# lionl1106/Clip-Neural-image-conpression

Hardware: AMD Instinct MI355X
Metric: images/sec @256px 50-step DDIM, batch=8/GPU (higher is better)
Workload: dtype bf16; 1 GPU; 256px base=128 ch_mult=(1, 2, 2) 50-step DDIM (eta=0), batch=8/GPU, key-seeded synthetic weights (out.* x0.1), synthetic z / x_T; global_batch=8, parallelism=dp1 (independent batches, no collective in the loop), graph=hipGraph, one replay per step, steps_in_flight=1

## Files before the change

clip-neural-image-conpression_amd/csrc/ccn_api.hip:

```cpp
#include "../../include/ccn_hip.h"
#include "ccn_internal.h"

#include <algorithm>
#include <cmath>
#include <cstdio>
#include <cstdlib>
#include <cstring>
#include <functional>
#include <map>
#include <memory>
#include <string>
#include <vector>

using namespace ccn;

namespace {

thread_local std::string g_err;
int fail(int code, const std::string& msg) { g_err = msg; return code; }
#define HIPCHK(expr)                                                                                     \
    do {                                                                                                 \
        hipError_t e_ = (expr);                                                                          \
        if (e_ != hipSuccess)                                                                            \
            return fail(CCN_EHIP, std::string(#expr) + ": " + hipGetErrorString(e_));                    \
// ... 314 lines not shown
        std::vector<uint16_t> buf(n, 0);
        for (int t = 0; t < taps; ++t)
            for (int o = 0; o < cw.Cout; ++o)
                for (int i = 0; i < cw.Cin_pad; ++i) buf[((size_t)t * cw.Cout_pad + o) * cw.Cin_pad + i] = f2bf_host(at(t, o, i));
        return upload(h, buf.data(), n * 2, &cw.w);
    }
    std::vector<float> buf(n, 0.f);
    for (int t = 0; t < taps; ++t)
        for (int o = 0; o < cw.Cout; ++o)
            for (int i = 0; i < cw.Cin_pad; ++i) buf[((size_t)t * cw.Cout_pad + o) * cw.Cin_pad + i] = at(t, o, i);
    return upload(h, buf.data(), n * 4, &cw.w);
}

int pack_conv3(ccn_handle_s* h, ConvW& cw, const std::string& name)
{
    const float* w = h->host.at(name + ".weight").data();
    const int cke = conv_cin_chunk(h->cfg.dtype);
    cw.Cin_pad = (int)align_up(cw.Cin, cke);
    const int I = cw.Cin;
    int rc = pack_and_upload(h, cw, 9, [&](int t, int o, int i) { return i < I ? w[((size_t)o * I + i) * 9 + t] : 0.f; });
    if (rc) return rc;
    if (cw.kind == KIND_C3S2 && cw.BN == 128 && h->cfg.dtype == CCN_DTYPE_BF16) {
        const int nch = cw.Cin_pad / cke, n32 = cw.Cout_pad / 32, O = cw.Cout;
        std::vector<uint16_t> fr((size_t)nch * 5 * n32 * 2 * 4 * 64 * 8, 0);
        for (int o = 0; o < O; ++o)
            for (int i = 0; i < I; ++i)
                for (int ps = 0; ps < 10; ++ps) {
                    const int tp = prs2_tap(ps >> 1, ps & 1);
                    if (tp >= 0) fr[prs2_frag_index(ps >> 1, ps & 1, o, i, cw.Cout_pad)] = f2bf_host(w[((size_t)o * I + i) * 9 + tp]);
                }
        if ((rc = upload(h, fr.data(), fr.size() * 2, &cw.wfrag))) return rc;
    }
    if (cw.kind == KIND_C3S1 && cw.BN == 128 && h->cfg.dtype == CCN_DTYPE_BF16) {
        const int nch = cw.Cin_pad / cke, n32 = cw.Cout_pad / 32, O = cw.Cout;
        std::vector<uint16_t> fr((size_t)nch * n32 * 36 * 64 * 8, 0);
        for (int o = 0; o < O; ++o)
            for (int i = 0; i < I; ++i)
                for (int t = 0; t < 9; ++t) fr[pr3_frag_index(o, i, t, cw.Cout_pad)] = f2bf_host(w[((size_t)o * I + i) * 9 + t]);
        if ((rc = upload(h, fr.data(), fr.size() * 2, &cw.wfrag))) return rc;
    }
    return upload_f32(h, name + ".bias", &cw.bias);
}
int pack_convT(ccn_handle_s* h, ConvW& cw, const std::string& name)
{
    const float* w = h->host.at(name + ".weight").data();
    const int cke = conv_cin_chunk(h->cfg.dtype);
    cw.Cin_pad = (int)align_up(cw.Cin, cke);
    const int I = cw.Cin, O = cw.Cout;
    int rc = pack_and_upload(h, cw, 16, [&](int t, int o, int i) { return i < I ? w[((size_t)i * O + o) * 16 + t] : 0.f; });
    if (rc) return rc;
    if (cw.BN == 128 && h->cfg.dtype == CCN_DTYPE_BF16) {
        const int nch = cw.Cin_pad / cke, n32 = cw.Cout_pad / 32;
        std::vector<uint16_t> fr((size_t)4 * nch * n32 * 4 * 4 * 64 * 8, 0);
// ... 29 lines not shown
    }
    return upload_f32(h, name + ".bias", &cw.bias);
}

struct PlanBuilder {
    ccn_handle_s* h;
    Plan* plan;
    Bump bump;
    int B;
    int film_stride;
    PlanBuilder(ccn_handle_s* h_, Plan* p, void* ws, bool measure) : h(h_), plan(p), bump(ws, measure), B(p->B), film_stride(h_->F) {}

    TensorRef new_tensor(int C, int H, int W)
    {
        TensorRef t; t.C = C; t.H = H; t.W = W;
        t.p = bump.take((size_t)B * H * W * C * h->elem);
        return t;
    }
    float2* new_ab(int C) { return (float2*)bump.take((size_t)B * C * sizeof(float2)); }
    int groups_for(int C) const { return C < h->G ? C : h->G; }

    ConvRoute route(const ConvW& cw, int Hin, int Win, bool gn_ab, bool res, bool film) const
    {
        static const ConvPolicy policy{true, 128, false, !diag_env("CCN_NO_SPLITK"), diag_env("CCN_SPLITK_S1") != nullptr, true};
        return conv_route({h->cfg.dtype, cw.kind, false, cw.BN, cw.Cin, cw.Cin_pad, cw.Cout, cw.Cout_pad, B, Hin, Win, h->G, cw.wfrag != nullptr,
                           gn_ab, res, film}, policy);
    }

    void conv(const ConvW& cw, int family, const TensorRef& in, TensorRef& out, const float2* gn_ab, int film_off,
              const TensorRef* res, bool want_part, bool is_stem = false, bool is_head = false, const NormW* in_norm = nullptr)
    {
        const ConvRoute r = route(cw, in.H, in.W, gn_ab != nullptr, res != nullptr, film_off >= 0);
        const ConvGeom& g = r.g;
        std::shared_ptr<ConvArgs> ap(new ConvArgs());
        ConvArgs& a = *ap;
        r.fill(a);
        a.in = in.p; a.w = cw.w; a.wfrag = r.uses_frag() ? cw.wfrag : nullptr; a.bias = cw.bias; a.out = out.p;
        a.film = nullptr; a.res = res ? res->p : nullptr;
        static const bool no_instat = diag_env("CCN_NO_INSTAT") != nullptr;
        if (in_norm) {
            const int G_in = groups_for(cw.Cin), cpg_in = cw.Cin / G_in;
            if (r.gs_ok && !no_instat && in.C == cw.Cin && conv_in_kernel_stats(h->cfg.dtype, in.C, G_in, in.n_sp, in.bn)) {
                a.gs_part = in.part; a.gs_gamma = in_norm->gamma; a.gs_beta = in_norm->beta;
                a.gs_inv_count = 1.0 / ((double)cpg_in * in.H * in.W);
                a.gs_nsp = in.n_sp; a.gs_nnt = in.n_nt; a.gs_bn = in.bn; a.gs_cpg = cpg_in;
            } else gn_ab = gn(in, *in_norm);
        }
// ... 814 lines not shown
```

clip-neural-image-conpression_amd/csrc/ccn_conv_pr.hip:

```cpp
#include "ccn_device.h"
#include <cstdio>
#include <cstdlib>
#include <cstring>
#include <vector>
#include <algorithm>

namespace ccn {

namespace {

#define CCN_FDIV(x, m, d) ((m) ? (int)__umulhi((unsigned)(x), (m)) : (int)(x))

template <int TH_> struct PrLdsT {
    static constexpr int HROWS = TH_ + 2, HPITCH = 34;
    static constexpr int A_BYTES = HROWS * HPITCH * 128;
    static constexpr int SP = 272;
    static constexpr int STG_BYTES = TH_ * 32 * SP;
    static constexpr int CHS_BYTES = 4 * 128 * 2 * 4;
    static constexpr int TOTAL = 2 * A_BYTES + STG_BYTES + CHS_BYTES;
};
typedef PrLdsT<8> PrLds;
static_assert(PrLds::TOTAL <= 160 * 1024, "LDS budget");

}

template <int NTAPS, int D, int MODE, int TH = 8, int GS = 0, bool P4 = false>
__global__ __launch_bounds__(512) void conv_pr_kernel(const ConvArgs a, const int grid_tiles)
{
    static_assert(TH == 8 || (TH == 4 && NTAPS == 9), "4-row tiles: 3x3 stride-1 form only");
    static_assert(!P4 || (NTAPS == 4 && MODE != 2), "plane passes of 2x2 taps: the 4-tap consumers, no split-K");
    constexpr bool RES = MODE == 1;
    constexpr bool RR = MODE != 0;
    typedef __bf16 T;
    constexpr int MF = 4, NF = 2;
    constexpr int BN = 128;
    constexpr int HROWS = TH + 2;
    constexpr int OSC = (NTAPS == 4 && !P4) ? 2 : 1, NPARC = (NTAPS == 4 && !P4) ? 4 : 1;
    constexpr int EPC = 8, CKE = 64;
    constexpr int NSTEP = NTAPS * 4;
    constexpr bool S2 = NTAPS == 2;
    constexpr int NPASS = S2 ? 5 : (P4 ? 4 : 1);
    constexpr int IS = (S2 || P4) ? 2 : 1;
    static_assert(NSTEP % D == 0, "the register ring must wrap at the chunk boundary");
    using L = PrLdsT<TH>;
    constexpr int HPITCH = L::HPITCH;
    extern __shared__ __attribute__((aligned(16))) unsigned char smem[];
    unsigned char* const stg = smem + 2 * L::A_BYTES;

    const int tid = threadIdx.x, lane = tid & 63, wave = tid >> 6;
    const int r = lane & 31, h = lane >> 5;

    const int grid = (int)gridDim.x;
    const int vb = (grid & 7) == 0 ? ((int)blockIdx.x & 7) * (grid >> 3) + ((int)blockIdx.x >> 3) : (int)blockIdx.x;
    const int ntiles = grid_tiles;
    const int my_tiles = (ntiles - vb + grid - 1) / grid;
    auto vt = [&](int ti) __attribute__((always_inline)) { return vb + ti * grid; };
    const int ks = (MODE == 2 && a.ksplit == 2) ? 2 : 1;
    const unsigned xcc_id = MODE == 2 ? (unsigned)__builtin_amdgcn_s_getreg((3 << 11) | 20) : 0u;
    const int nck = a.nchunk / ks;
    const int ktotal = my_tiles * nck;
    auto vt_tile = [&](int v) __attribute__((always_inline)) { return ks == 2 ? (v >> 1) : v; };
    auto vt_kh = [&](int v) __attribute__((always_inline)) { return ks == 2 ? (v & 1) : 0; };

    const unsigned char* const inb = (const unsigned char*)a.in;
    constexpr bool gstat = GS == 1;
    static_assert(GS != 1 || (NTAPS == 9 && MODE != 2), "in-kernel statistics: 3x3 stride-1 layers without split-K");
// ... 282 lines not shown
            qn_bt[0] = *(const f32x4*)(a.gs_beta + q_cbs); qn_bt[1] = *(const f32x4*)(a.gs_beta + q_cbs + 4);
        } else gkn.load(a.gn_ab + (size_t)q_b * a.Cin + q_cbs, gn && q_cv);
    };
    auto coef_sel = [&]() __attribute__((always_inline)) {
        if (gstat) {
            const int src = CCN_FDIV(q_cbs, a.fd_gscpg, a.gs_cpg) * 8;
            qn_mean = __shfl(st_mean, src); qn_rstd = __shfl(st_rstd, src);
        }
    };
    auto prep = [&]() __attribute__((always_inline)) {
        const bool fresh = decode();
        coef_loads();
        if (fresh) { stats_issue(q_b); stats_reduce(); st_b = q_b; }
        coef_sel();
    };
    auto adopt = [&]() __attribute__((always_inline)) {
        if (gstat) gk.from_raw(qn_g, qn_bt, qn_mean, qn_rstd, gn && q_cv_i);
        else gk = gkn;
    };
    auto issue_loads = [&](int r0 = 0, int r1 = TH + 2, bool with_x = true) __attribute__((always_inline)) {
        const int b = __builtin_amdgcn_readfirstlane(q_b), iy0 = __builtin_amdgcn_readfirstlane(q_iy0), ix0 = __builtin_amdgcn_readfirstlane(q_ix0);
        const int cc = __builtin_amdgcn_readfirstlane(q_c / NPASS);
        const int pass = q_c - cc * NPASS;
        const int py = S2 ? (pass <= 2 ? 1 : 0) : (P4 ? (pass < 2 ? 1 : 0) : 0);
        const int px = S2 ? ((pass <= 1 || pass == 3) ? 1 : 0) : (P4 ? ((pass & 1) ? 0 : 1) : 0);
        const int cb = cc * CKE + ck * EPC;
        const bool cv = q_tv && cb < a.Cin;
        q_cv_i = cv;
        const unsigned img_bytes = (unsigned)(a.Hin * a.Win * a.Cin) * (unsigned)sizeof(T);
        const unsigned coff = (unsigned)(((q_tv && cc * CKE < a.Cin) ? cc : 0) * CKE) * (unsigned)sizeof(T);
        const auto srd = __builtin_amdgcn_make_buffer_rsrc((void*)(inb + (size_t)b * img_bytes + coff), 0, img_bytes - coff, 0x00020000);
        const int rs = IS * a.Win * a.Cin * (int)sizeof(T);
        const int ixr = IS * (ix0 + pcol) + px;
        colv = cv && ixr >= 0 && ixr < a.Win;
        const unsigned cmask = colv ? 0u : OOB;
        const int base = ((IS * iy0 + py) * a.Win + ixr) * a.Cin * (int)sizeof(T) + ck * 16;
        const int first = IS * iy0 + py;
        const int r_lo = first < 0 ? (-first + IS - 1) / IS : 0;
        int r_hi = (a.Hin - first + IS - 1) / IS; r_hi = r_hi > HROWS ? HROWS : (r_hi < 0 ? 0 : r_hi);
        rowm = q_tv ? (((1u << r_hi) - 1u) & ~((1u << r_lo) - 1u)) : 0u;
#pragma unroll
        for (int i = 0; i < HROWS; ++i) {
            if (i < r0 || i >= r1) continue;
            areg[i] = __builtin_amdgcn_raw_buffer_load_b128(srd, (unsigned)(base + i * rs) | cmask, 0, 0);
        }
        {
            const int iyr = IS * (iy0 + xrow) + py, ixx = IS * (ix0 + xcol) + px;
            xv = xthr && cv && iyr >= 0 && iyr < a.Hin && ixx >= 0 && ixx < a.Win;
// ... 175 lines not shown
                    for (int i = 0; i < TH; ++i)
#pragma unroll
                        for (int q = 0; q < 4; ++q) {
                            const f32x16& c = acc[i];
                            typedef unsigned u32x2 __attribute__((ext_vector_type(2)));
                            const u32x2 pk = {pack_bf2(c[q * 4], c[q * 4 + 1]), pack_bf2(c[q * 4 + 2], c[q * 4 + 3])};
                            *(u32x2*)(stg + stg_lane + (i * 32 + (q >> 1) * 16) * L::SP + ((q & 1) * 16) * 2) = pk;
                        }
                }
                timed_barrier();
            }
        }
        __builtin_amdgcn_s_setprio(0);
        stamp(2); stamp_cycles();
    } else {
    static_assert(TH == 8, "the 4x2 fragment form works on 8-row tiles");
    const int wm = wave >> 1, wn = wave & 1;
    f32x16 acc[MF][NF];
    auto rbase = [&](int row_lin, int hx) __attribute__((always_inline)) { return row_lin * 128 + (((hx >> 1) & 6) << 4) + (((h ^ (hx >> 1)) & 1) << 4); };
    int prow[MF];
#pragma unroll
    for (int i = 0; i < MF; ++i) prow[i] = ((wm * MF + i) + 1) * HPITCH + r + 1;
    const int n32 = a.Cout_pad / 32;
    constexpr unsigned COLB = NSTEP * 1024;
    const unsigned wtotal = (unsigned)((size_t)NPARC * a.nchunk * n32 * COLB);
    const auto wsrd = __builtin_amdgcn_make_buffer_rsrc((void*)a.wfrag, 0, wtotal, 0x00020000);
    const unsigned lane16 = (unsigned)lane * 16u;
    auto wbase_of = [&](int tile, int chunk) __attribute__((always_inline)) -> unsigned {
        const int t2 = CCN_FDIV(tile, a.fd_nt, a.n_nt);
        const int nt = tile - t2 * a.n_nt, par = t2 % NPARC;
        return (unsigned)__builtin_amdgcn_readfirstlane((int)((unsigned)((par * a.nchunk + chunk) * n32 + nt * 4 + wn * NF) * COLB));
    };
    u32x4 bq[D][NF];
    {
        const unsigned wb = wbase_of(vt_tile(vt(0)), vt_kh(vt(0)) * nck);
#pragma unroll
        for (int s = 0; s < D - 1; ++s)
#pragma unroll
            for (int jn = 0; jn < NF; ++jn) bq[s][jn] = __builtin_amdgcn_raw_buffer_load_b128(wsrd, lane16, wb + s * 1024 + jn * COLB, 0);
    }
    const int stg_lane = (wm * 4 * 32 + r) * L::SP + (wn * 64 + 4 * h) * 2;

    if constexpr (HSPLIT < HROWS) {
        request_first(HSPLIT, HROWS, false);
        dump(0, HSPLIT, HROWS, false);
    }
    raw_barrier();
    stamp(1);
    int k = 0;
    for (int ti = 0; ti < my_tiles; ++ti) {
        const int v = vt(ti), v_next = ti + 1 < my_tiles ? vt(ti + 1) : v;
        const int tile = vt_tile(v), c0 = vt_kh(v) * nck;
        int toffs[NTAPS], tdxs[NTAPS];
        if constexpr (NTAPS == 4 && !P4) {
            const int par = CCN_FDIV(tile, a.fd_nt, a.n_nt) % NPARC;
#pragma unroll
            for (int t = 0; t < NTAPS; ++t) { tdxs[t] = a.tapinfo_dx(par * 4 + t); toffs[t] = a.tapinfo_dy(par * 4 + t) * HPITCH + tdxs[t]; }
        }
#pragma unroll
        for (int i = 0; i < MF; ++i)
#pragma unroll
            for (int j = 0; j < NF; ++j)
#pragma unroll
                for (int q = 0; q < 16; ++q) acc[i][j][q] = 0.0f;
        for (int chunk = 0; chunk < nck; ++chunk, ++k) {
            const unsigned wb_cur = wbase_of(tile, c0 + chunk);
            const unsigned wb_nxt = chunk + 1 < nck ? wbase_of(tile, c0 + chunk + 1) : wbase_of(vt_tile(v_next), vt_kh(v_next) * nck);
            const int bufoff = (k & 1) * L::A_BYTES;
            if constexpr (S2) {
                const int pass = (c0 + chunk) % 5;
                tdxs[0] = (pass == 0 || pass == 1 || pass == 3) ? -1 : 0; tdxs[1] = 0;
                toffs[0] = ((pass == 0 || pass == 2) ? -HPITCH : 0) + tdxs[0];
                toffs[1] = pass == 0 ? -HPITCH : 0;
            }
            if constexpr (P4) {
                const int pass = (c0 + chunk) & 3;
                const int py = pass < 2 ? 1 : 0, px = (pass & 1) ? 0 : 1;
#pragma unroll
                for (int t = 0; t < NTAPS; ++t) { tdxs[t] = (t & 1) - px; toffs[t] = ((t >> 1) - py) * HPITCH + tdxs[t]; }
            }
#pragma unroll
            for (int i = 0; i < MF; ++i) asm volatile("" : "+v"(prow[i]));
            u32x4 av[2][MF];
            int abase[MF];
            auto frag = [&](int j, u32x4* av_) __attribute__((always_inline)) {
                const int tt = j >> 2, kk = j & 3;
                if (kk == 0) {
#pragma unroll
                    for (int i = 0; i < MF; ++i) abase[i] = bufoff + rbase(prow[i] + toffs[tt], r + 1 + tdxs[tt]);
                }
#pragma unroll
                for (int i = 0; i < MF; ++i) av_[i] = *(const u32x4*)(smem + (abase[i] ^ (kk << 5)));
            };
            if (!CCN_DBG_BIT(a, 64)) {
            frag(0, av[0]);
#pragma unroll
            for (int j = 0; j < NSTEP; ++j) {
                __builtin_amdgcn_sched_barrier(0);
                {
                    const int p = j + D - 1;
                    const unsigned off = p < NSTEP ? wb_cur + (unsigned)p * 1024u : wb_nxt + (unsigned)(p - NSTEP) * 1024u;
#pragma unroll
                    for (int jn = 0; jn < NF; ++jn)
                        bq[p % D][jn] = __builtin_amdgcn_raw_buffer_load_b128(wsrd, lane16, off + jn * COLB, 0);
                }
                if (j + 1 < NSTEP) frag(j + 1, av[(j + 1) & 1]);
#pragma unroll
                for (int jn = 0; jn < NF; ++jn)
#pragma unroll
                    for (int ii = 0; ii < MF; ++ii) { const int i = (jn & 1) ? MF - 1 - ii : ii; mfma16<T>(acc[i][jn], bq[j % D][jn], av[j & 1][i]); }
#pragma unroll
                for (int m = 0; m < MF * NF; ++m) {
                    __builtin_amdgcn_sched_group_barrier(0x008, 1, 0);
                    if (m < NF) __builtin_amdgcn_sched_group_barrier(0x020, 1, 0);
                    __builtin_amdgcn_sched_group_barrier(0x100, 1, 0);
                    __builtin_amdgcn_sched_group_barrier(0x002, 2, 0);
                }
                __builtin_amdgcn_sched_barrier(0);
            }
            }
            if (chunk + 1 == nck) {
#pragma unroll
                for (int i = 0; i < MF; ++i)
#pragma unroll
                    for (int j = 0; j < NF; ++j)
#pragma unroll
                        for (int g = 0; g < 4; ++g) {
                            const f32x16& c = acc[i][j];
                            typedef unsigned u32x2 __attribute__((ext_vector_type(2)));
                            const u32x2 pk = {pack_bf2(c[g * 4], c[g * 4 + 1]), pack_bf2(c[g * 4 + 2], c[g * 4 + 3])};
                            *(u32x2*)(stg + stg_lane + i * 32 * L::SP + (j * 32 + g * 8) * 2) = pk;
                        }
            }
            timed_barrier();
        }
    }
    __builtin_amdgcn_s_setprio(0);
    stamp(2); stamp_cycles();
    }
}

constexpr int PR_D = 6;
typedef void (*pr_fn_t)(const ConvArgs, int);
static pr_fn_t pick_pr(int ntaps, int mode, int th = 8, int gs = 0)
{
    if (ntaps == 16) return mode == 1 ? (pr_fn_t)conv_pr_kernel<4, 8, 1, 8, 0, true> : (pr_fn_t)conv_pr_kernel<4, 8, 0, 8, 0, true>;
    if (gs == 1 && ntaps == 9 && mode != 2) {
        if (th == 4) return mode == 1 ? (pr_fn_t)conv_pr_kernel<9, PR_D, 1, 4, 1> : (pr_fn_t)conv_pr_kernel<9, PR_D, 0, 4, 1>;
        return mode == 1 ? (pr_fn_t)conv_pr_kernel<9, PR_D, 1, 8, 1> : (pr_fn_t)conv_pr_kernel<9, PR_D, 0, 8, 1>;
    }
    if (gs == 2 && ntaps == 9) {
        if (th == 4) return mode == 1 ? (pr_fn_t)conv_pr_kernel<9, PR_D, 1, 4, 2> : (mode == 2 ? (pr_fn_t)conv_pr_kernel<9, PR_D, 2, 4, 2> : (pr_fn_t)conv_pr_kernel<9, PR_D, 0, 4, 2>);
        return mode == 1 ? (pr_fn_t)conv_pr_kernel<9, PR_D, 1, 8, 2> : (mode == 2 ? (pr_fn_t)conv_pr_kernel<9, PR_D, 2, 8, 2> : (pr_fn_t)conv_pr_kernel<9, PR_D, 0, 8, 2>);
    }
    if (ntaps == 9 && th == 4) return mode == 1 ? (pr_fn_t)conv_pr_kernel<9, PR_D, 1, 4> : (mode == 2 ? (pr_fn_t)conv_pr_kernel<9, PR_D, 2, 4> : (pr_fn_t)conv_pr_kernel<9, PR_D, 0, 4>);
    if (ntaps == 9) return mode == 1 ? (pr_fn_t)conv_pr_kernel<9, PR_D, 1> : (mode == 2 ? (pr_fn_t)conv_pr_kernel<9, PR_D, 2> : (pr_fn_t)conv_pr_kernel<9, PR_D, 0>);
    if (ntaps == 2) return mode == 1 ? (pr_fn_t)conv_pr_kernel<2, 8, 1> : (mode == 2 ? (pr_fn_t)conv_pr_kernel<2, 8, 2> : (pr_fn_t)conv_pr_kernel<2, 8, 0>);
    return mode == 1 ? (pr_fn_t)conv_pr_kernel<4, 8, 1> : (mode == 2 ? (pr_fn_t)conv_pr_kernel<4, 8, 2> : (pr_fn_t)conv_pr_kernel<4, 8, 0>);
}

bool conv_pr_supported(int kind, int bn, int th)
{
    return bn == 128 && (((kind == KIND_C3S1 || kind == KIND_CT4 || kind == KIND_C3S2) && th == 8) || (kind == KIND_C3S1 && th == 4));
}

static int g_cus = 0;
hipError_t conv_pr_prepare()
{
    hipError_t e = hipSuccess;
    for (int ntaps : {2, 4, 9, 16})
        for (int mode = 0; mode < 3; ++mode) {
            if (ntaps == 16 && mode == 2) continue;
            e = hipFuncSetAttribute((const void*)pick_pr(ntaps, mode), hipFuncAttributeMaxDynamicSharedMemorySize, (int)PrLds::TOTAL);
            if (e != hipSuccess) return e;
        }
    for (int mode = 0; mode < 3; ++mode) {
        e = hipFuncSetAttribute((const void*)pick_pr(9, mode, 4), hipFuncAttributeMaxDynamicSharedMemorySize, (int)PrLdsT<4>::TOTAL);
        if (e != hipSuccess) return e;
    }
    for (int gs = 1; gs <= 2; ++gs)
// ... 12 lines not shown
    if (e != hipSuccess) return e;
    g_cus = prop.multiProcessorCount;
    return hipSuccess;
}

static unsigned long long* g_stamps = nullptr;
static unsigned g_stamp_grid = 0;
extern "C" int ccn_internal_dump_stamps_pr(const char* path)
{
    if (!g_stamps || !g_stamp_grid) return 1;
    std::vector<unsigned long long> hbuf((size_t)g_stamp_grid * 16);
    if (hipMemcpy(hbuf.data(), g_stamps, hbuf.size() * 8, hipMemcpyDeviceToHost) != hipSuccess) return 2;
    FILE* f = fopen(path, "w");
    if (!f) return 3;
    for (unsigned b = 0; b < g_stamp_grid; ++b)
        for (int k = 0; k < 16; ++k) fprintf(f, "%llu%c", hbuf[(size_t)b * 16 + k], k == 15 ? '\n' : ' ');
    fclose(f);
    return 0;
}

hipError_t launch_conv_pr(int dtype, const ConvArgs& a, hipStream_t s)
{
    const bool c3 = a.ntaps == 9 && a.npar == 1 && a.OS == 1, ct = a.ntaps == 4 && a.npar == 4 && a.OS == 2;
    const bool s2 = a.ntaps == 2 && a.npar == 1 && a.OS == 1 && !a.gn_ab && (a.nchunk % 5) == 0;
    const bool p4 = a.ntaps == 16 && a.npar == 1 && a.OS == 1 && (a.nchunk % 4) == 0 && a.ksplit != 2;
    if ((ct || s2 || p4) && (a.gn_ab || a.gs_part)) return hipErrorInvalidValue;
    if (dtype != 1 || !a.wfrag || !(c3 || ct || s2 || p4) || !(a.th == 8 || (a.th == 4 && c3)) || (a.Cout_pad & 127) || a.nchunk < 2 || a.fin_counter || (a.res && a.film)) return hipErrorInvalidValue;
    const int ks = a.ksplit == 2 ? 2 : 1;
    if (ks == 2 && (!a.kpart || !a.kflag || (a.nchunk & 1) || (s2 && (a.nchunk / 2) % 5) || a.res)) return hipErrorInvalidValue;
    const int ntiles = a.B * a.n_ty * a.n_tx * a.npar * a.n_nt * ks;
    static const int cap = diag_env("CCN_PR_GRID") ? atoi(diag_env("CCN_PR_GRID")) : 0;
    int grid = cap > 0 ? cap : (g_cus > 0 ? g_cus : 256);
    if (grid > ntiles) grid = ntiles;
    if (ks == 2) { grid &= ~15; if (grid < 16) return hipErrorInvalidValue; }
    ConvArgs d = a;
    {
        auto magic = [](long dv) -> unsigned { return dv <= 1 ? 0u : (unsigned)((0x100000000ull + (unsigned long long)dv - 1) / (unsigned long long)dv); };
        const long dmax = std::max<long>(std::max<long>((long)a.n_nt * a.npar, (long)a.n_tx * a.n_ty), std::max<long>(a.cpg, a.gs_cpg));
        if ((unsigned long long)std::max<long>(ntiles, 8192) * (unsigned long long)dmax >= 0x100000000ull) return hipErrorInvalidValue;
        d.fd_nt = magic(a.n_nt); d.fd_ntp = magic((long)a.n_nt * a.npar); d.fd_tx = magic(a.n_tx); d.fd_sp = magic((long)a.n_tx * a.n_ty);
        d.fd_cpg = magic(a.cpg); d.fd_gscpg = magic(a.gs_cpg);
        d.fd_gsbn = magic(a.gs_bn); d.fd_gsnsp = magic(a.gs_nsp);
    }
    d.prod_first = (a.nchunk <= 2 && c3) ? 1 : 0;
    static const char* env = diag_env("CCN_STAMPS");
    if (env && (unsigned)atoi(env) == (unsigned)ntiles && (!strchr(env, ':') || atoi(strchr(env, ':') + 1) == a.ntaps)) {
        if (!g_stamps) { if (hipMalloc((void**)&g_stamps, (size_t)1024 * 24 * 8) != hipSuccess) return hipErrorOutOfMemory; }
        g_stamp_grid = (unsigned)grid;
        d.stamps = g_stamps;
    } else d.stamps = nullptr;
    if (a.gs_part && !(c3 && ks == 1)) return hipErrorInvalidValue;
    hipLaunchKernelGGL(pick_pr(a.ntaps, a.res ? 1 : (ks == 2 ? 2 : 0), a.th, a.gs_part ? 1 : (a.gn_ab ? 0 : 2)), dim3((unsigned)grid), dim3(512),
// ... 6 lines not shown
```

clip-neural-image-conpression_amd/csrc/ccn_internal.h:

```cpp
#pragma once
#include <hip/hip_runtime.h>
#include <stdint.h>
#include <stddef.h>

#include <stdlib.h>

#ifdef CCN_DIAG
#define CCN_DBG_BIT(a, bit) ((((a).dbg) & (bit)) != 0)
#define CCN_STAMPS_PTR(a) ((a).stamps)
namespace ccn { inline const char* diag_env(const char* name) { return getenv(name); } }
#else
#define CCN_DBG_BIT(a, bit) false
#define CCN_STAMPS_PTR(a) ((unsigned long long*)nullptr)
namespace ccn { inline const char* diag_env(const char*) { return nullptr; } }
#endif

namespace ccn {

__host__ __device__ inline int pr3_slice(int g, int k32) { return ((g & 1) << 2) | (k32 << 1) | (g >> 1); }
__host__ __device__ inline size_t pr3_frag_index(int n, int k, int t, int Np)
{
    const int chunk = k >> 6, s = (k & 63) >> 3, e = k & 7;
    const int g = ((s >> 2) & 1) | ((s & 1) << 1), k32 = (s >> 1) & 1;
    const int nn = n >> 5, c = (n >> 4) & 1, lane = g * 16 + (n & 15);
    const int dy = t / 3, dx = t - dy * 3;
    const int f = ((dx * 2 + k32) * 3 + dy) * 2 + c;
    return ((((size_t)chunk * (size_t)(Np >> 5) + nn) * 36 + f) * 64 + lane) * 8 + e;
}

__host__ __device__ inline size_t pr4_frag_elem(size_t group, int n, int k)
{
    const int kw = k & 63;
    return ((group * 4 + (size_t)(kw >> 4)) * 64 + (size_t)((((kw >> 3) & 1) << 5) | (n & 31))) * 8 + (size_t)(kw & 7);
}
__host__ __device__ inline int prct_tap(int par, int t)
{
    const int ky = (par >> 1) ? ((t >> 1) ? 2 : 0) : ((t >> 1) ? 3 : 1), kx = (par & 1) ? ((t & 1) ? 2 : 0) : ((t & 1) ? 3 : 1);
    return ky * 4 + kx;
}
__host__ __device__ inline size_t prct_frag_index(int par, int t, int n, int k, int Np, int nch)
{
    return pr4_frag_elem((((size_t)par * nch + (k >> 6)) * (size_t)(Np >> 5) + (n >> 5)) * 4 + t, n, k);
}
__host__ __device__ inline int prs2_tap(int pass, int slot)
{
    const int dy = pass == 0 ? 0 : (pass == 1 ? 2 : (pass == 2 ? (slot ? 2 : 0) : 1));
    const int dx = pass == 2 ? 1 : (pass == 4 ? 1 : (slot ? 2 : 0));
    return (pass == 4 && slot) ? -1 : dy * 3 + dx;
}
__host__ __device__ inline size_t prs2_frag_index(int pass, int slot, int n, int k, int Np)
{
    return pr4_frag_elem((((size_t)(k >> 6) * 5 + pass) * (size_t)(Np >> 5) + (n >> 5)) * 2 + slot, n, k);
}
__host__ __device__ inline int prp4_tap(int pass, int t)
{
    const int py = pass < 2 ? 1 : 0, px = (pass & 1) ? 0 : 1, i = t >> 1, j = t & 1;
    const int ky = py ? (i ? 2 : 0) : (i ? 3 : 1), kx = px ? (j ? 2 : 0) : (j ? 3 : 1);
    return ky * 4 + kx;
}
__host__ __device__ inline size_t prp4_frag_index(int pass, int t, int n, int k, int Np)
{
    return pr4_frag_elem((((size_t)(k >> 6) * 4 + pass) * (size_t)(Np >> 5) + (n >> 5)) * 4 + t, n, k);
}

enum ConvKind { KIND_C3S1 = 0, KIND_C3S2 = 1, KIND_CT4 = 2, KIND_STEM = 3, KIND_HEAD = 4 };

struct ConvArgs {
    const void* in;
    const void* w;
    const void* wfrag;
    const float* bias;
    void* out;
    const float2* gn_ab;
    const float2* gs_part;
    const float* gs_gamma; const float* gs_beta;
// ... 131 lines not shown
```

clip-neural-image-conpression_amd/csrc/ccn_kernels.hip:

```cpp
#include "ccn_device.h"
#include <cstdlib>

namespace ccn {

__host__ __device__ constexpr int cmax(int a, int b) { return a > b ? a : b; }

template <int AK, int IS> struct HaloGeom {
    static constexpr int HOFF = AK == A_NHWC ? 1 : 0;
    static constexpr int ROWS = AK == A_NHWC ? (IS == 1 ? 6 : 10) : 4;
    static constexpr int PITCH = AK == A_NHWC ? (IS == 1 ? 34 : 66) : 32;
    static constexpr int BYTES = ROWS * PITCH * 128;
};
template <int AK, int IS, int BN> struct LdsGeom {
    static constexpr int A_BYTES = HaloGeom<AK, IS>::BYTES;
    static constexpr int B_BYTES = BN * 128;
    static constexpr int CP = BN + 4;
    static constexpr int CS_BYTES = 128 * CP * 4;
    static constexpr int RED_BYTES = 4 * BN * 2 * 4 + BN * 2 * 4;
    static constexpr int TOTAL = cmax(A_BYTES + 2 * B_BYTES, CS_BYTES + RED_BYTES);
};

template <typename T, int AK, int IS, int EPI, int WM, int WN, int MF, int NF>
__global__ __launch_bounds__(256) void conv_igemm_kernel(const ConvArgs a)
{
// ... 413 lines not shown
    const int k = four ? 4 : 3;
    for (int ky = 0; ky < k; ++ky)
        for (int kx = 0; kx < k; ++kx) tapinfo[ky * k + kx] = ConvArgs::make_tap(ky - 1, kx - 1, ky * k + kx);
}

ConvRoute conv_route(const ConvQuery& q, const ConvPolicy& p)
{
    ConvRoute r{};
    r.q = q;
    r.n_nt = q.Cout_pad / q.BN;
    const ConvGeom g8 = conv_geom(q.kind, q.four, q.Hin, q.Win, 8);
    const long tiles8 = (long)q.B * g8.n_ty * g8.n_tx * g8.npar * r.n_nt;
    r.th = conv_tile_rows(q.kind, q.BN, q.B, g8.MH, g8.MW, g8.npar, r.n_nt);
    const int nch = q.Cin_pad / conv_cin_chunk(q.dtype);
    const double out_bytes = (double)q.B * g8.Hout * g8.Wout * q.Cout * (q.dtype == 1 ? 2 : 4);
    if (p.pr && q.frag && nch >= 2 && !(q.res && q.film) && out_bytes < 2.0e9) {
        if (q.kind == KIND_C3S1) r.pr = conv_pr_selected(q.dtype, q.kind, q.BN, r.th);
        else if (!q.gn_ab && (q.kind == KIND_C3S2 || (q.kind == KIND_CT4 && !q.four))) {
            if (q.kind == KIND_CT4 && !p.ct_like_s2) r.pr = conv_pr_selected(q.dtype, q.kind, q.BN, r.th);
            else if (conv_pr_selected(q.dtype, q.kind, q.BN, 8) && tiles8 >= p.s2_min_tiles8) { r.pr = true; r.th = 8; }
        }
    }
    r.ksplit = 1;
    if (r.pr && p.split_k && !q.res && (q.kind == KIND_C3S2 || (q.kind == KIND_C3S1 && p.split_k_s1))) {
        const int nk = q.kind == KIND_C3S2 ? 5 * nch : nch;
        if (tiles8 >= 32 && tiles8 <= 128 && nk >= 4 && (nch & 1) == 0) { r.ksplit = 2; r.th = 8; }
    }
    r.g = conv_geom(q.kind, q.four, q.Hin, q.Win, r.th);
    r.nchunk = nch; r.ntaps = r.g.ntaps;
    if (r.pr && q.kind == KIND_C3S2) {
        if (q.four) r.nchunk *= 4;
        else { r.nchunk *= 5; r.ntaps = 2; }
    }
    r.gs_ok = r.pr && r.ksplit == 1 && q.kind == KIND_C3S1;
    r.fin_blocks = r.g.n_ty * r.g.n_tx * r.g.npar * r.n_nt;
    r.nslot = r.fin_blocks;
    r.part_nsp = r.g.n_ty * r.g.n_tx * r.g.npar; r.part_nnt = r.n_nt; r.part_bn = q.BN;
    r.stem2 = p.stem2 && q.kind == KIND_STEM && q.frag && stem2_supported(q.dtype, q.Cin, q.Cout, q.G) && !q.gn_ab && !q.film && !q.res;
    if (r.stem2) {
        r.nslot = 4 * stem2_blocks(q.Hin, q.Win, nullptr);
        r.part_nsp = r.nslot; r.part_nnt = 1; r.part_bn = 1 << 30;
    }
    return r;
}

void ConvRoute::fill(ConvArgs& a) const
{
    a.B = q.B; a.Hin = q.Hin; a.Win = q.Win; a.Cin = q.Cin; a.Cin_pad = q.Cin_pad;
    a.Hout = g.Hout; a.Wout = g.Wout; a.Cout = q.Cout; a.Cout_pad = q.Cout_pad;
    a.MH = g.MH; a.MW = g.MW; a.OS = g.OS; a.npar = g.npar; a.ntaps = ntaps;
    a.th = th; a.n_ty = g.n_ty; a.n_tx = g.n_tx; a.n_nt = n_nt; a.nchunk = nchunk;
    a.use_pr = pr ? 1 : 0; a.use_stem2 = stem2 ? 1 : 0; a.ksplit = ksplit;
    a.silu = 1;
    a.G = q.Cout < q.G ? q.Cout : q.G; a.cpg = q.Cout / a.G;
    a.nslot = nslot; a.fin_blocks = fin_blocks; a.bn = q.BN;
// ... 376 lines not shown
```

clip-neural-image-conpression_amd/csrc/ccn_train.hip:

```cpp
#include "../../include/ccn_hip.h"
#include "ccn_train.h"

#include <climits>
#include <cmath>
#include <cstdio>
#include <cstdlib>
#include <cstring>
#include <map>
#include <string>
#include <vector>

using namespace ccn;

extern "C" void ccn_internal_set_error(const char* msg);

namespace {

int tfail(int code, const std::string& msg) { ccn_internal_set_error(msg.c_str()); return code; }
#define THIP(expr)                                                                                       \
    do {                                                                                                 \
        hipError_t e_ = (expr);                                                                          \
        if (e_ != hipSuccess) { err = std::string(#expr) + ": " + hipGetErrorString(e_); return false; } \
    } while (0)

// ... 165 lines not shown
    w.dCin_pad = w.dkind == KIND_STEM ? cke : (int)align_up(w.Cout, cke);
    if (!alloc_dev(tr, (size_t)w.dtaps * w.dCout_pad * w.dCin_pad * tr->elem, &w.wd, err)) return false;
    switch (fkind) {
        case KIND_C3S1: w.pd_d = {src, w.wd, PK_DG3S1, w.Cout, w.Cin, 9, w.dCout_pad, w.dCin_pad}; break;
        case KIND_C3S2: w.pd_d = {src, w.wd, PK_DG3S2, w.Cout, w.Cin, 16, w.dCout_pad, w.dCin_pad}; break;
        case KIND_CT4: w.pd_d = {src, w.wd, PK_DGT, w.Cout, w.Cin, 16, w.dCout_pad, w.dCin_pad}; break;
        case KIND_HEAD: w.pd_d = {src, w.wd, PK_HEAD_DG, w.Cout, w.Cin, 1, w.dCout_pad, w.dCin_pad}; break;
    }
    if (fkind == KIND_HEAD && stem2_supported(tr->cfg.dtype, w.Cout, w.Cin, tr->G)) {
        if (!alloc_dev(tr, (size_t)w.Cin * 32 * 2, &w.wd_frag, err)) return false;
        w.pf_d = {src, w.wd_frag, PK_FRAG_STEM_HEAD_DG, w.Cout, w.Cin, 1, w.Cin, 32, 0};
    }
    if (fkind == KIND_C3S1 && tr->elem == 2) {
        if (w.BN == 128 && w.Cin_pad >= 128) {
            if (!alloc_dev(tr, (size_t)9 * w.Cout_pad * w.Cin_pad * 2, &w.wf_frag, err)) return false;
            w.pf_f = {src, w.wf_frag, PK_FRAG3, w.Cout, w.Cin, 9, w.Cout_pad, w.Cin_pad};
        }
        if (w.dBN == 128 && w.dCin_pad >= 128) {
            if (!alloc_dev(tr, (size_t)9 * w.dCout_pad * w.dCin_pad * 2, &w.wd_frag, err)) return false;
            w.pf_d = {src, w.wd_frag, PK_FRAG3_DG, w.Cout, w.Cin, 9, w.dCout_pad, w.dCin_pad};
        }
    }
    if (tr->elem == 2 && (fkind == KIND_C3S2 || fkind == KIND_CT4) && w.BN == 128 && w.Cin_pad >= 128) {
        const int slots = fkind == KIND_C3S2 ? 10 : 16;
        if (!alloc_dev(tr, (size_t)slots * w.Cout_pad * w.Cin_pad * 2, &w.wf_frag, err)) return false;
        w.pf_f = {src, w.wf_frag, fkind == KIND_C3S2 ? PK_FRAG_S2 : PK_FRAG_CT, w.Cout, w.Cin, slots, w.Cout_pad, w.Cin_pad};
    }
    if (tr->elem == 2 && (fkind == KIND_C3S2 || fkind == KIND_CT4) && w.dBN == 128 && w.dCin_pad >= 128) {
        if (!alloc_dev(tr, (size_t)16 * w.dCout_pad * w.dCin_pad * 2, &w.wd_frag, err)) return false;
        w.pf_d = {src, w.wd_frag, fkind == KIND_C3S2 ? PK_FRAG_CT_DG : PK_FRAG_P4_DG, w.Cout, w.Cin, 16, w.dCout_pad, w.dCin_pad};
    }
    return true;
}

struct Walk {
    ccn_trainer_s* tr;
    int B, H, W;
    char* base; size_t off = 0;
    bool launch;
    hipStream_t st;
    const float* P; float* Gd;
    ShapeInfo need;
    float *scr_wg = nullptr, *scr_col = nullptr; float2 *scr_gn = nullptr, *scr_film = nullptr;
    std::string err;
    float *temb = nullptr, *u0 = nullptr, *t1 = nullptr, *tp = nullptr, *uz = nullptr, *zpv = nullptr, *hv = nullptr, *film = nullptr;
    float *dfilm = nullptr, *dh = nullptr, *dt1 = nullptr, *du0 = nullptr, *duz = nullptr;
    struct ResSave { TT x, y, o, xa, ya; bool pre = false; float2 *ab1, *st1, *ab2, *st2; };
// ... 783 lines not shown
```

clip-neural-image-conpression_amd/csrc/ccn_train_kernels.hip:

```cpp
#include "ccn_device.h"
#include "ccn_train.h"
#include <cstdlib>

namespace ccn {

namespace {
template <typename T> __device__ __forceinline__ T to_elem(float v);
template <> __device__ __forceinline__ float to_elem<float>(float v) { return v; }
template <> __device__ __forceinline__ __bf16 to_elem<__bf16>(float v) { return (__bf16)v; }
template <typename T> __device__ __forceinline__ float from_elem(T v) { return (float)v; }

template <typename T> __device__ __forceinline__ float dsilu(float y);
template <> __device__ __forceinline__ float dsilu<float>(float y) { const float sg = 1.0f / (1.0f + expf(-y)); return sg * (1.0f + y * (1.0f - sg)); }
template <> __device__ __forceinline__ float dsilu<__bf16>(float y) { const float sg = __builtin_amdgcn_rcpf(1.0f + __expf(-y)); return sg * (1.0f + y * (1.0f - sg)); }

template <typename T> struct Chunk {
    static constexpr int E = 8;
    static __device__ __forceinline__ void load(const T* p, float* v);
    static __device__ __forceinline__ void store(T* p, const float* v);
};
template <> __device__ __forceinline__ void Chunk<float>::load(const float* p, float* v) {
    const f32x4 a = *(const f32x4*)p, b = *(const f32x4*)(p + 4);
#pragma unroll
    for (int e = 0; e < 4; ++e) { v[e] = a[e]; v[4 + e] = b[e]; }
// ... 63 lines not shown
                    if (n < I && k < O) { const float* p = w + ((size_t)k * I + n) * 9;
#pragma unroll
                        for (int t = 0; t < 9; ++t) v[e][(t / 3) * 4 + (t % 3)] = p[t]; }
                } else {
                    if (n < I && k < O) { const float* p = w + ((size_t)n * O + k) * 16;
#pragma unroll
                        for (int t = 0; t < 16; ++t) v[e][t] = p[t]; }
                }
            }
            auto piece = [&](int tp) __attribute__((always_inline)) -> u32x4 {
                u32x4 r = {0u, 0u, 0u, 0u};
                if (tp >= 0) {
#pragma unroll
                    for (int q = 0; q < 4; ++q) r[q] = pack_bf2(v[2 * q][tp], v[2 * q + 1][tp]);
                }
                return r;
            };
            unsigned short* const db = (unsigned short*)dst;
            if (mode == PK_FRAG3 || mode == PK_FRAG3_DG) {
#pragma unroll
                for (int t = 0; t < 9; ++t) *(u32x4*)(db + pr3_frag_index(n, k0, t, Np)) = piece(t);
            } else if (mode == PK_FRAG_S2) {
#pragma unroll
                for (int ps = 0; ps < 10; ++ps) *(u32x4*)(db + prs2_frag_index(ps >> 1, ps & 1, n, k0, Np)) = piece(prs2_tap(ps >> 1, ps & 1));
            } else if (mode == PK_FRAG_P4_DG) {
#pragma unroll
                for (int pt = 0; pt < 16; ++pt) *(u32x4*)(db + prp4_frag_index(pt >> 2, pt & 3, n, k0, Np)) = piece(prp4_tap(pt >> 2, pt & 3));
            } else {
#pragma unroll
                for (int pt = 0; pt < 16; ++pt) *(u32x4*)(db + prct_frag_index(pt >> 2, pt & 3, n, k0, Np, Kp >> 6)) = piece(prct_tap(pt >> 2, pt & 3));
            }
        }
        return;
    }
    for (size_t idx = (size_t)blockIdx.x * blockDim.x + threadIdx.x; idx < plane; idx += (size_t)gridDim.x * blockDim.x) {
        const int k = (int)(idx % Kp), n = (int)(idx / Kp);
        float v[16];
#pragma unroll
        for (int t = 0; t < 16; ++t) v[t] = 0.f;
        switch (d.mode) {
            case PK_CONV3:
                if (n < O && k < I) { const float* p = w + ((size_t)n * I + k) * 9;
#pragma unroll
                    for (int t = 0; t < 9; ++t) v[t] = p[t]; }
                break;
            case PK_CONVT:
                if (n < O && k < I) { const float* p = w + ((size_t)k * O + n) * 16;
// ... 28 lines not shown
            case PK_FRAG_S2:
                if (n < O && k < I) { const float* p = w + ((size_t)n * I + k) * 9;
#pragma unroll
                    for (int t = 0; t < 9; ++t) v[t] = p[t]; }
                break;
            case PK_FRAG_CT:
                if (n < O && k < I) { const float* p = w + ((size_t)k * O + n) * 16;
#pragma unroll
                    for (int t = 0; t < 16; ++t) v[t] = p[t]; }
                break;
            case PK_FRAG_P4_DG:
                if (n < I && k < O) { const float* p = w + ((size_t)n * O + k) * 16;
#pragma unroll
                    for (int t = 0; t < 16; ++t) v[t] = p[t]; }
                break;
            case PK_FRAG_CT_DG:
                if (n < I && k < O) { const float* p = w + ((size_t)k * I + n) * 9;
#pragma unroll
                    for (int t = 0; t < 16; ++t) v[t] = ((t >> 2) < 3 && (t & 3) < 3) ? p[(t >> 2) * 3 + (t & 3)] : 0.f; }
                break;
        }
        if (d.mode == PK_FRAG_S2) {
#pragma unroll
            for (int ps = 0; ps < 10; ++ps) {
                const int tp = prs2_tap(ps >> 1, ps & 1);
                float val = 0.f;
#pragma unroll
                for (int t = 0; t < 9; ++t) val = t == tp ? v[t] : val;
                dst[prs2_frag_index(ps >> 1, ps & 1, n, k, Np)] = to_elem<T>(val);
            }
            continue;
        }
        if (d.mode == PK_FRAG_P4_DG) {
#pragma unroll
            for (int pt = 0; pt < 16; ++pt) {
                const int tp = prp4_tap(pt >> 2, pt & 3);
                float val = 0.f;
#pragma unroll
                for (int t = 0; t < 16; ++t) val = t == tp ? v[t] : val;
                dst[prp4_frag_index(pt >> 2, pt & 3, n, k, Np)] = to_elem<T>(val);
            }
            continue;
        }
        if (d.mode == PK_FRAG_CT || d.mode == PK_FRAG_CT_DG) {
#pragma unroll
            for (int pt = 0; pt < 16; ++pt) {
                const int tp = prct_tap(pt >> 2, pt & 3);
                float val = 0.f;
#pragma unroll
                for (int t = 0; t < 16; ++t) val = t == tp ? v[t] : val;
                dst[prct_frag_index(pt >> 2, pt & 3, n, k, Np, Kp >> 6)] = to_elem<T>(val);
            }
// ... 1168 lines not shown
```

Before: 83.97 images/sec.

## Restructure stride-2 conv into four phase planes with nine packed tap slots

The stride-2 3x3 polyphase conv previously ran five passes of two tap slots each, one of them zero-padded (ten slots, wasting one MMA step). It now uses four input-phase planes carrying 4/2/2/1 taps, packs the weights as nine contiguous slots per chunk, and processes all four planes of a chunk in one 36-step iteration, swapping LDS buffers at plane boundaries. This removes the padded tap's MMAs and weight traffic and lets the weight prefetch ring run across passes. Split-K for stride-2 convs is also switched from on-by-default to opt-in. That changes the tile scheduling and could lower occupancy on smaller layers.

```diff
diff --git a/clip-neural-image-conpression_amd/csrc/ccn_api.hip b/clip-neural-image-conpression_amd/csrc/ccn_api.hip
--- a/clip-neural-image-conpression_amd/csrc/ccn_api.hip
+++ b/clip-neural-image-conpression_amd/csrc/ccn_api.hip
@@ -360,13 +360,10 @@
     if (rc) return rc;
     if (cw.kind == KIND_C3S2 && cw.BN == 128 && h->cfg.dtype == CCN_DTYPE_BF16) {
         const int nch = cw.Cin_pad / cke, n32 = cw.Cout_pad / 32, O = cw.Cout;
-        std::vector<uint16_t> fr((size_t)nch * 5 * n32 * 2 * 4 * 64 * 8, 0);
+        std::vector<uint16_t> fr((size_t)nch * n32 * 9 * 4 * 64 * 8, 0);
         for (int o = 0; o < O; ++o)
             for (int i = 0; i < I; ++i)
-                for (int ps = 0; ps < 10; ++ps) {
-                    const int tp = prs2_tap(ps >> 1, ps & 1);
-                    if (tp >= 0) fr[prs2_frag_index(ps >> 1, ps & 1, o, i, cw.Cout_pad)] = f2bf_host(w[((size_t)o * I + i) * 9 + tp]);
-                }
+                for (int ps = 0; ps < 9; ++ps) fr[prs2_frag_index(ps, o, i, cw.Cout_pad)] = f2bf_host(w[((size_t)o * I + i) * 9 + prs2_tap(ps)]);
         if ((rc = upload(h, fr.data(), fr.size() * 2, &cw.wfrag))) return rc;
     }
     if (cw.kind == KIND_C3S1 && cw.BN == 128 && h->cfg.dtype == CCN_DTYPE_BF16) {
@@ -442,7 +439,7 @@
 
     ConvRoute route(const ConvW& cw, int Hin, int Win, bool gn_ab, bool res, bool film) const
     {
-        static const ConvPolicy policy{true, 128, false, !diag_env("CCN_NO_SPLITK"), diag_env("CCN_SPLITK_S1") != nullptr, true};
+        static const ConvPolicy policy{true, 128, false, diag_env("CCN_SPLITK") != nullptr, diag_env("CCN_SPLITK_S1") != nullptr, true};
         return conv_route({h->cfg.dtype, cw.kind, false, cw.BN, cw.Cin, cw.Cin_pad, cw.Cout, cw.Cout_pad, B, Hin, Win, h->G, cw.wfrag != nullptr,
                            gn_ab, res, film}, policy);
     }
diff --git a/clip-neural-image-conpression_amd/csrc/ccn_conv_pr.hip b/clip-neural-image-conpression_amd/csrc/ccn_conv_pr.hip
--- a/clip-neural-image-conpression_amd/csrc/ccn_conv_pr.hip
+++ b/clip-neural-image-conpression_amd/csrc/ccn_conv_pr.hip
@@ -39,9 +39,10 @@
     constexpr int EPC = 8, CKE = 64;
     constexpr int NSTEP = NTAPS * 4;
     constexpr bool S2 = NTAPS == 2;
-    constexpr int NPASS = S2 ? 5 : (P4 ? 4 : 1);
+    constexpr int NPASS = (S2 || P4) ? 4 : 1;
     constexpr int IS = (S2 || P4) ? 2 : 1;
-    static_assert(NSTEP % D == 0, "the register ring must wrap at the chunk boundary");
+    constexpr int NPC = S2 ? NPASS : 1, GSTEPS = S2 ? 36 : NSTEP;
+    static_assert(GSTEPS % D == 0, "the register ring must wrap at the iteration boundary");
     using L = PrLdsT<TH>;
     constexpr int HPITCH = L::HPITCH;
     extern __shared__ __attribute__((aligned(16))) unsigned char smem[];
@@ -370,8 +371,8 @@
         const int b = __builtin_amdgcn_readfirstlane(q_b), iy0 = __builtin_amdgcn_readfirstlane(q_iy0), ix0 = __builtin_amdgcn_readfirstlane(q_ix0);
         const int cc = __builtin_amdgcn_readfirstlane(q_c / NPASS);
         const int pass = q_c - cc * NPASS;
-        const int py = S2 ? (pass <= 2 ? 1 : 0) : (P4 ? (pass < 2 ? 1 : 0) : 0);
-        const int px = S2 ? ((pass <= 1 || pass == 3) ? 1 : 0) : (P4 ? ((pass & 1) ? 0 : 1) : 0);
+        const int py = (S2 || P4) ? (pass < 2 ? 1 : 0) : 0;
+        const int px = (S2 || P4) ? ((pass & 1) ? 0 : 1) : 0;
         const int cb = cc * CKE + ck * EPC;
         const bool cv = q_tv && cb < a.Cin;
         q_cv_i = cv;
@@ -593,14 +594,15 @@
 #pragma unroll
     for (int i = 0; i < MF; ++i) prow[i] = ((wm * MF + i) + 1) * HPITCH + r + 1;
     const int n32 = a.Cout_pad / 32;
-    constexpr unsigned COLB = NSTEP * 1024;
-    const unsigned wtotal = (unsigned)((size_t)NPARC * a.nchunk * n32 * COLB);
+    constexpr unsigned COLB = GSTEPS * 1024;
+    const int nwch = a.nchunk / NPC;
+    const unsigned wtotal = (unsigned)((size_t)NPARC * nwch * n32 * COLB);
     const auto wsrd = __builtin_amdgcn_make_buffer_rsrc((void*)a.wfrag, 0, wtotal, 0x00020000);
     const unsigned lane16 = (unsigned)lane * 16u;
     auto wbase_of = [&](int tile, int chunk) __attribute__((always_inline)) -> unsigned {
         const int t2 = CCN_FDIV(tile, a.fd_nt, a.n_nt);
         const int nt = tile - t2 * a.n_nt, par = t2 % NPARC;
-        return (unsigned)__builtin_amdgcn_readfirstlane((int)((unsigned)((par * a.nchunk + chunk) * n32 + nt * 4 + wn * NF) * COLB));
+        return (unsigned)__builtin_amdgcn_readfirstlane((int)((unsigned)((par * nwch + chunk / NPC) * n32 + nt * 4 + wn * NF) * COLB));
     };
     u32x4 bq[D][NF];
     {
@@ -634,16 +636,10 @@
             for (int j = 0; j < NF; ++j)
 #pragma unroll
                 for (int q = 0; q < 16; ++q) acc[i][j][q] = 0.0f;
-        for (int chunk = 0; chunk < nck; ++chunk, ++k) {
+        for (int chunk = 0; chunk < nck; chunk += NPC, k += NPC) {
             const unsigned wb_cur = wbase_of(tile, c0 + chunk);
-            const unsigned wb_nxt = chunk + 1 < nck ? wbase_of(tile, c0 + chunk + 1) : wbase_of(vt_tile(v_next), vt_kh(v_next) * nck);
-            const int bufoff = (k & 1) * L::A_BYTES;
-            if constexpr (S2) {
-                const int pass = (c0 + chunk) % 5;
-                tdxs[0] = (pass == 0 || pass == 1 || pass == 3) ? -1 : 0; tdxs[1] = 0;
-                toffs[0] = ((pass == 0 || pass == 2) ? -HPITCH : 0) + tdxs[0];
-                toffs[1] = pass == 0 ? -HPITCH : 0;
-            }
+            const unsigned wb_nxt = chunk + NPC < nck ? wbase_of(tile, c0 + chunk + NPC) : wbase_of(vt_tile(v_next), vt_kh(v_next) * nck);
+            int bufoff = (k & 1) * L::A_BYTES;
             if constexpr (P4) {
                 const int pass = (c0 + chunk) & 3;
                 const int py = pass < 2 ? 1 : 0, px = (pass & 1) ? 0 : 1;
@@ -657,25 +653,33 @@
             auto frag = [&](int j, u32x4* av_) __attribute__((always_inline)) {
                 const int tt = j >> 2, kk = j & 3;
                 if (kk == 0) {
-#pragma unroll
-                    for (int i = 0; i < MF; ++i) abase[i] = bufoff + rbase(prow[i] + toffs[tt], r + 1 + tdxs[tt]);
+                    int toff = 0, tdx = 0;
+                    if constexpr (S2) {
+                        const int tp = prs2_tap(tt);
+                        tdx = tp % 3 == 0 ? -1 : 0; toff = (tp < 3 ? -HPITCH : 0) + tdx;
+#pragma unroll
+                        for (int i = 0; i < MF; ++i) asm volatile("" : "+v"(prow[i]));
+                    } else { toff = toffs[tt]; tdx = tdxs[tt]; }
+#pragma unroll
+                    for (int i = 0; i < MF; ++i) abase[i] = bufoff + rbase(prow[i] + toff, r + 1 + tdx);
                 }
 #pragma unroll
                 for (int i = 0; i < MF; ++i) av_[i] = *(const u32x4*)(smem + (abase[i] ^ (kk << 5)));
             };
+            auto pass_end = [&](int j) __attribute__((always_inline)) -> bool { return S2 && (j == 15 || j == 23 || j == 31); };
             if (!CCN_DBG_BIT(a, 64)) {
             frag(0, av[0]);
 #pragma unroll
-            for (int j = 0; j < NSTEP; ++j) {
+            for (int j = 0; j < GSTEPS; ++j) {
                 __builtin_amdgcn_sched_barrier(0);
                 {
                     const int p = j + D - 1;
-                    const unsigned off = p < NSTEP ? wb_cur + (unsigned)p * 1024u : wb_nxt + (unsigned)(p - NSTEP) * 1024u;
+                    const unsigned off = p < GSTEPS ? wb_cur + (unsigned)p * 1024u : wb_nxt + (unsigned)(p - GSTEPS) * 1024u;
 #pragma unroll
                     for (int jn = 0; jn < NF; ++jn)
                         bq[p % D][jn] = __builtin_amdgcn_raw_buffer_load_b128(wsrd, lane16, off + jn * COLB, 0);
                 }
-                if (j + 1 < NSTEP) frag(j + 1, av[(j + 1) & 1]);
+                if (j + 1 < GSTEPS && !pass_end(j)) frag(j + 1, av[(j + 1) & 1]);
 #pragma unroll
                 for (int jn = 0; jn < NF; ++jn)
 #pragma unroll
@@ -688,9 +692,16 @@
                     __builtin_amdgcn_sched_group_barrier(0x002, 2, 0);
                 }
                 __builtin_amdgcn_sched_barrier(0);
-            }
-            }
-            if (chunk + 1 == nck) {
+                if (pass_end(j)) {
+                    timed_barrier();
+                    bufoff = L::A_BYTES - bufoff;
+                    frag(j + 1, av[(j + 1) & 1]);
+                }
+            }
+            } else {
+                for (int pp = 1; pp < NPC; ++pp) timed_barrier();
+            }
+            if (chunk + NPC == nck) {
 #pragma unroll
                 for (int i = 0; i < MF; ++i)
 #pragma unroll
@@ -726,7 +737,7 @@
     }
     if (ntaps == 9 && th == 4) return mode == 1 ? (pr_fn_t)conv_pr_kernel<9, PR_D, 1, 4> : (mode == 2 ? (pr_fn_t)conv_pr_kernel<9, PR_D, 2, 4> : (pr_fn_t)conv_pr_kernel<9, PR_D, 0, 4>);
     if (ntaps == 9) return mode == 1 ? (pr_fn_t)conv_pr_kernel<9, PR_D, 1> : (mode == 2 ? (pr_fn_t)conv_pr_kernel<9, PR_D, 2> : (pr_fn_t)conv_pr_kernel<9, PR_D, 0>);
-    if (ntaps == 2) return mode == 1 ? (pr_fn_t)conv_pr_kernel<2, 8, 1> : (mode == 2 ? (pr_fn_t)conv_pr_kernel<2, 8, 2> : (pr_fn_t)conv_pr_kernel<2, 8, 0>);
+    if (ntaps == 2) return mode == 1 ? (pr_fn_t)conv_pr_kernel<2, PR_D, 1> : (mode == 2 ? (pr_fn_t)conv_pr_kernel<2, PR_D, 2> : (pr_fn_t)conv_pr_kernel<2, PR_D, 0>);
     return mode == 1 ? (pr_fn_t)conv_pr_kernel<4, 8, 1> : (mode == 2 ? (pr_fn_t)conv_pr_kernel<4, 8, 2> : (pr_fn_t)conv_pr_kernel<4, 8, 0>);
 }
 
@@ -785,12 +796,12 @@
 hipError_t launch_conv_pr(int dtype, const ConvArgs& a, hipStream_t s)
 {
     const bool c3 = a.ntaps == 9 && a.npar == 1 && a.OS == 1, ct = a.ntaps == 4 && a.npar == 4 && a.OS == 2;
-    const bool s2 = a.ntaps == 2 && a.npar == 1 && a.OS == 1 && !a.gn_ab && (a.nchunk % 5) == 0;
+    const bool s2 = a.ntaps == 2 && a.npar == 1 && a.OS == 1 && !a.gn_ab && (a.nchunk % 4) == 0;
     const bool p4 = a.ntaps == 16 && a.npar == 1 && a.OS == 1 && (a.nchunk % 4) == 0 && a.ksplit != 2;
     if ((ct || s2 || p4) && (a.gn_ab || a.gs_part)) return hipErrorInvalidValue;
     if (dtype != 1 || !a.wfrag || !(c3 || ct || s2 || p4) || !(a.th == 8 || (a.th == 4 && c3)) || (a.Cout_pad & 127) || a.nchunk < 2 || a.fin_counter || (a.res && a.film)) return hipErrorInvalidValue;
     const int ks = a.ksplit == 2 ? 2 : 1;
-    if (ks == 2 && (!a.kpart || !a.kflag || (a.nchunk & 1) || (s2 && (a.nchunk / 2) % 5) || a.res)) return hipErrorInvalidValue;
+    if (ks == 2 && (!a.kpart || !a.kflag || (a.nchunk & 1) || (s2 && (a.nchunk / 2) % 4) || a.res)) return hipErrorInvalidValue;
     const int ntiles = a.B * a.n_ty * a.n_tx * a.npar * a.n_nt * ks;
     static const int cap = diag_env("CCN_PR_GRID") ? atoi(diag_env("CCN_PR_GRID")) : 0;
     int grid = cap > 0 ? cap : (g_cus > 0 ? g_cus : 256);
diff --git a/clip-neural-image-conpression_amd/csrc/ccn_internal.h b/clip-neural-image-conpression_amd/csrc/ccn_internal.h
--- a/clip-neural-image-conpression_amd/csrc/ccn_internal.h
+++ b/clip-neural-image-conpression_amd/csrc/ccn_internal.h
@@ -42,15 +42,15 @@
 {
     return pr4_frag_elem((((size_t)par * nch + (k >> 6)) * (size_t)(Np >> 5) + (n >> 5)) * 4 + t, n, k);
 }
-__host__ __device__ inline int prs2_tap(int pass, int slot)
-{
-    const int dy = pass == 0 ? 0 : (pass == 1 ? 2 : (pass == 2 ? (slot ? 2 : 0) : 1));
-    const int dx = pass == 2 ? 1 : (pass == 4 ? 1 : (slot ? 2 : 0));
-    return (pass == 4 && slot) ? -1 : dy * 3 + dx;
-}
-__host__ __device__ inline size_t prs2_frag_index(int pass, int slot, int n, int k, int Np)
-{
-    return pr4_frag_elem((((size_t)(k >> 6) * 5 + pass) * (size_t)(Np >> 5) + (n >> 5)) * 2 + slot, n, k);
+__host__ __device__ inline int prs2_tap(int slot)
+{
+    const int dy = slot < 4 ? ((slot >> 1) << 1) : (slot < 6 ? (slot - 4) << 1 : 1);
+    const int dx = slot < 4 ? ((slot & 1) << 1) : (slot < 6 ? 1 : (slot < 8 ? (slot - 6) << 1 : 1));
+    return dy * 3 + dx;
+}
+__host__ __device__ inline size_t prs2_frag_index(int slot, int n, int k, int Np)
+{
+    return pr4_frag_elem((((size_t)(k >> 6) * (size_t)(Np >> 5) + (n >> 5)) * 9 + slot), n, k);
 }
 __host__ __device__ inline int prp4_tap(int pass, int t)
 {
diff --git a/clip-neural-image-conpression_amd/csrc/ccn_kernels.hip b/clip-neural-image-conpression_amd/csrc/ccn_kernels.hip
--- a/clip-neural-image-conpression_amd/csrc/ccn_kernels.hip
+++ b/clip-neural-image-conpression_amd/csrc/ccn_kernels.hip
@@ -459,15 +459,15 @@
         }
     }
     r.ksplit = 1;
-    if (r.pr && p.split_k && !q.res && (q.kind == KIND_C3S2 || (q.kind == KIND_C3S1 && p.split_k_s1))) {
-        const int nk = q.kind == KIND_C3S2 ? 5 * nch : nch;
+    if (r.pr && !q.res && ((q.kind == KIND_C3S2 && p.split_k) || (q.kind == KIND_C3S1 && p.split_k_s1))) {
+        const int nk = q.kind == KIND_C3S2 ? 4 * nch : nch;
         if (tiles8 >= 32 && tiles8 <= 128 && nk >= 4 && (nch & 1) == 0) { r.ksplit = 2; r.th = 8; }
     }
     r.g = conv_geom(q.kind, q.four, q.Hin, q.Win, r.th);
     r.nchunk = nch; r.ntaps = r.g.ntaps;
     if (r.pr && q.kind == KIND_C3S2) {
         if (q.four) r.nchunk *= 4;
-        else { r.nchunk *= 5; r.ntaps = 2; }
+        else { r.nchunk *= 4; r.ntaps = 2; }
     }
     r.gs_ok = r.pr && r.ksplit == 1 && q.kind == KIND_C3S1;
     r.fin_blocks = r.g.n_ty * r.g.n_tx * r.g.npar * r.n_nt;
diff --git a/clip-neural-image-conpression_amd/csrc/ccn_train.hip b/clip-neural-image-conpression_amd/csrc/ccn_train.hip
--- a/clip-neural-image-conpression_amd/csrc/ccn_train.hip
+++ b/clip-neural-image-conpression_amd/csrc/ccn_train.hip
@@ -211,7 +211,7 @@
         }
     }
     if (tr->elem == 2 && (fkind == KIND_C3S2 || fkind == KIND_CT4) && w.BN == 128 && w.Cin_pad >= 128) {
-        const int slots = fkind == KIND_C3S2 ? 10 : 16;
+        const int slots = fkind == KIND_C3S2 ? 9 : 16;
         if (!alloc_dev(tr, (size_t)slots * w.Cout_pad * w.Cin_pad * 2, &w.wf_frag, err)) return false;
         w.pf_f = {src, w.wf_frag, fkind == KIND_C3S2 ? PK_FRAG_S2 : PK_FRAG_CT, w.Cout, w.Cin, slots, w.Cout_pad, w.Cin_pad};
     }
diff --git a/clip-neural-image-conpression_amd/csrc/ccn_train_kernels.hip b/clip-neural-image-conpression_amd/csrc/ccn_train_kernels.hip
--- a/clip-neural-image-conpression_amd/csrc/ccn_train_kernels.hip
+++ b/clip-neural-image-conpression_amd/csrc/ccn_train_kernels.hip
@@ -109,7 +109,7 @@
                 for (int t = 0; t < 9; ++t) *(u32x4*)(db + pr3_frag_index(n, k0, t, Np)) = piece(t);
             } else if (mode == PK_FRAG_S2) {
 #pragma unroll
-                for (int ps = 0; ps < 10; ++ps) *(u32x4*)(db + prs2_frag_index(ps >> 1, ps & 1, n, k0, Np)) = piece(prs2_tap(ps >> 1, ps & 1));
+                for (int ps = 0; ps < 9; ++ps) *(u32x4*)(db + prs2_frag_index(ps, n, k0, Np)) = piece(prs2_tap(ps));
             } else if (mode == PK_FRAG_P4_DG) {
 #pragma unroll
                 for (int pt = 0; pt < 16; ++pt) *(u32x4*)(db + prp4_frag_index(pt >> 2, pt & 3, n, k0, Np)) = piece(prp4_tap(pt >> 2, pt & 3));
@@ -184,12 +184,12 @@
         }
         if (d.mode == PK_FRAG_S2) {
 #pragma unroll
-            for (int ps = 0; ps < 10; ++ps) {
-                const int tp = prs2_tap(ps >> 1, ps & 1);
+            for (int ps = 0; ps < 9; ++ps) {
+                const int tp = prs2_tap(ps);
                 float val = 0.f;
 #pragma unroll
                 for (int t = 0; t < 9; ++t) val = t == tp ? v[t] : val;
-                dst[prs2_frag_index(ps >> 1, ps & 1, n, k, Np)] = to_elem<T>(val);
+                dst[prs2_frag_index(ps, n, k, Np)] = to_elem<T>(val);
             }
             continue;
         }
```

New measurement: 83.31 images/sec (median of 2 runs). Within noise of the previous version (-0.8%).
